# taichi-dev/taichi-nerfs

Hardware: NVIDIA H100
Metric: rays/sec (8192-ray batch, Lego shape) (higher is better)
Workload: dtype f16

## Files before the change

taichi_nerfs_b200/csrc/hash.cu:

```cuda
#include "common.cuh"

namespace {

constexpr int kTile = 512;
constexpr int kChunk = 16;
constexpr int kThreads = 512;
constexpr int kRow = kTile + kTile / kChunk + 1;
constexpr int kXChunk = kChunk + 1;
constexpr int kXWords = (kTile / kChunk) * kXChunk * 4;

struct Dyn {
    const int32_t* n_dev;
    float lo[3], span[3];
    int normalize;
};
__device__ __forceinline__ int64_t effective_n(const Dyn& dyn, int64_t n) {
    if (dyn.n_dev == nullptr) return n;
    const int64_t v = (int64_t)*dyn.n_dev;
    return v < n ? (v < 0 ? 0 : v) : n;
}

struct LevelMeta {
    uint32_t offset;
    uint32_t size;
    uint32_t mask;
    uint32_t res, res2;
    float scale;
    int dense;
};

__device__ __forceinline__ LevelMeta level_meta(const ngp_hash_layout& lay, int l) {
    LevelMeta m;
    m.offset = (uint32_t)lay.offsets[l];
    m.size = (uint32_t)lay.map_sizes[l];
    m.mask = (m.size & (m.size - 1)) == 0 ? m.size - 1 : 0u;
    m.res = lay.resolutions[l];
    m.res2 = m.res * m.res;
    m.scale = lay.scales[l];
    m.dense = l < lay.begin_fast_hash_level;
    return m;
}

template <bool kFracF16>
__device__ __forceinline__ void grid_pos(const float x[3], const LevelMeta& m, uint32_t g[3], float pos[3]) {
#pragma unroll
    for (int d = 0; d < 3; ++d) {
        const float p = f_add(f_mul(x[d], m.scale), 0.5f);
        const float fl = floorf(p);
        g[d] = (uint32_t)(int32_t)fl;
        const float gf = kFracF16 ? __half2float(__float2half_rn((float)g[d])) : (float)g[d];
        pos[d] = f_sub(p, gf);
    }
}

__device__ __forceinline__ void corner_indices(const LevelMeta& m, const uint32_t g[3], uint32_t idx[8]) {
    if (m.dense) {
        const uint32_t base = g[0] + g[1] * m.res + g[2] * m.res2;
#pragma unroll
        for (int c = 0; c < 8; ++c) {
            uint32_t h = base + (c & 1) + ((c >> 1) & 1) * m.res + (c >> 2) * m.res2;
            if (h >= m.size) {
                h -= m.size;
                if (h >= m.size) h %= m.size;
            }
            idx[c] = m.offset + h;
        }
    } else {
        const uint32_t hy0 = g[1] * 2654435761u, hy1 = hy0 + 2654435761u;
        const uint32_t hz0 = g[2] * 805459861u, hz1 = hz0 + 805459861u;
#pragma unroll
        for (int c = 0; c < 8; ++c) {
            const uint32_t h = (g[0] + (c & 1)) ^ ((c & 2) ? hy1 : hy0) ^ ((c & 4) ? hz1 : hz0);
            idx[c] = m.offset + (m.mask ? (h & m.mask) : (h % m.size));
        }
    }
}

__device__ __forceinline__ void corner_weights(const float pos[3], float w[8]) {
    const float ax[2] = {f_sub(1.0f, pos[0]), pos[0]};
    const float ay[2] = {f_sub(1.0f, pos[1]), pos[1]};
    const float az[2] = {f_sub(1.0f, pos[2]), pos[2]};
    float axy[4];
#pragma unroll
    for (int c = 0; c < 4; ++c) axy[c] = f_mul(ax[c & 1], ay[c >> 1]);
#pragma unroll
    for (int c = 0; c < 8; ++c) w[c] = f_mul(axy[c & 3], az[c >> 2]);
}

template <typename T>
struct Vec2;
template <>
struct Vec2<float> { using type = float2; };
template <>
struct Vec2<__half> { using type = __half2; };

template <typename V2>
struct Pair;
template <>
struct Pair<float2> {
    using type = float4;
    __device__ static __forceinline__ float2 lo(const float4& p) { return make_float2(p.x, p.y); }
    __device__ static __forceinline__ float2 hi(const float4& p) { return make_float2(p.z, p.w); }
};
template <>
struct Pair<__half2> {
    using type = uint2;
    __device__ static __forceinline__ __half2 lo(const uint2& p) { return *reinterpret_cast<const __half2*>(&p.x); }
    __device__ static __forceinline__ __half2 hi(const uint2& p) { return *reinterpret_cast<const __half2*>(&p.y); }
};

template <typename T>
__global__ void __launch_bounds__(kThreads) hash_fwd_kernel(const float* __restrict__ xyz,
                                                            const T* __restrict__ table,
                                                            const __grid_constant__ ngp_hash_layout lay,
                                                            T* __restrict__ out, int64_t n_max, const Dyn dyn) {
    using V2 = typename Vec2<T>::type;
    const int64_t n = effective_n(dyn, n_max);
    constexpr bool kHalf = sizeof(T) == 2;
    extern __shared__ __align__(16) uint8_t smem_raw[];
    float* sx = reinterpret_cast<float*>(smem_raw);
    V2* tile = reinterpret_cast<V2*>(smem_raw + kXWords * sizeof(float));

    const int L = lay.n_levels;
    const int64_t base = (int64_t)blockIdx.x * kTile;
    if (base >= n) return;
    const int rows = (int)min((int64_t)kTile, n - base);
    for (int r = threadIdx.x; r < rows; r += kThreads) {
        float v[3];
#pragma unroll
        for (int k = 0; k < 3; ++k) {
            v[k] = xyz[(base + r) * 3 + k];
            if (dyn.normalize) v[k] = f_div(f_sub(v[k], dyn.lo[k]), dyn.span[k]);
        }
        reinterpret_cast<float4*>(sx)[r + r / kChunk] = make_float4(v[0], v[1], v[2], 0.0f);
    }
    __syncthreads();

    const int level = threadIdx.x >> 5, lane = threadIdx.x & 31;
    if (level < L) {
        const LevelMeta m = level_meta(lay, level);
        const V2* tab = reinterpret_cast<const V2*>(table);
        uint32_t pg[3] = {0u, 0u, 0u};
        bool have = false;
        V2 v[8];
        V2* trow = tile + level * kRow + lane * (kChunk + 1);
#pragma unroll 4
        for (int j = 0; j < kChunk; ++j) {
            const int s = lane * kChunk + j;
            if (s >= rows) break;
            const float4 xv = reinterpret_cast<const float4*>(sx)[lane * kXChunk + j];
            const float x[3] = {xv.x, xv.y, xv.z};
            uint32_t g[3];
            float pos[3];
            grid_pos<kHalf>(x, m, g, pos);
            if (!have || g[0] != pg[0] || g[1] != pg[1] || g[2] != pg[2]) {
                have = true;
                uint32_t idx[8];
                corner_indices(m, g, idx);
#pragma unroll
                for (int c = 0; c < 8; c += 2) {
                    if ((idx[c] ^ idx[c + 1]) == 1u) {
                        using V4 = typename Pair<V2>::type;
                        const V4 pr = __ldg(reinterpret_cast<const V4*>(tab + (idx[c] & ~1u)));
                        const V2 lo = Pair<V2>::lo(pr), hi = Pair<V2>::hi(pr);
                        v[c] = (idx[c] & 1u) ? hi : lo;
                        v[c + 1] = (idx[c] & 1u) ? lo : hi;
                    } else {
                        v[c] = __ldg(tab + idx[c]);
                        v[c + 1] = __ldg(tab + idx[c + 1]);
                    }
                }
                pg[0] = g[0];
                pg[1] = g[1];
                pg[2] = g[2];
            }
            float w[8];
            corner_weights(pos, w);
            if constexpr (kHalf) {
                __half2 acc = __float2half2_rn(0.0f);
#pragma unroll
                for (int c = 0; c < 8; ++c) {
                    const float2 t = __half22float2(v[c]);
                    acc = __hadd2(acc, __floats2half2_rn(f_mul(w[c], t.x), f_mul(w[c], t.y)));
                }
                trow[j] = acc;
            } else {
                float2 acc = make_float2(0.0f, 0.0f);
#pragma unroll
                for (int c = 0; c < 8; ++c) {
                    acc.x = f_add(acc.x, f_mul(w[c], v[c].x));
                    acc.y = f_add(acc.y, f_mul(w[c], v[c].y));
                }
                trow[j] = acc;
            }
        }
    }
    __syncthreads();
    V2* o2 = reinterpret_cast<V2*>(out) + base * L;
    constexpr int kVec = 16 / sizeof(V2);
    if (L % kVec == 0 && (reinterpret_cast<uintptr_t>(out) & 15) == 0) {
        const int groups = L / kVec;
        for (int k = threadIdx.x; k < rows * groups; k += kThreads) {
            const int r = k / groups, l0 = (k - r * groups) * kVec;
            V2 v[kVec];
#pragma unroll
            for (int q = 0; q < kVec; ++q) v[q] = tile[(l0 + q) * kRow + r + r / kChunk];
            *reinterpret_cast<uint4*>(o2 + (int64_t)r * L + l0) = *reinterpret_cast<const uint4*>(v);
        }
    } else {
        for (int k = threadIdx.x; k < rows * L; k += kThreads) {
            const int r = k / L, l = k - r * L;
            o2[k] = tile[l * kRow + r + r / kChunk];
        }
    }
}

template <typename T>
__global__ void __launch_bounds__(kThreads) hash_bwd_kernel(const float* __restrict__ xyz,
                                                            const T* __restrict__ dout,
                                                            const __grid_constant__ ngp_hash_layout lay,
                                                            float* __restrict__ grad_table, int64_t n_max,
                                                            const Dyn dyn, int level_begin, int level_end,
                                                            int32_t* __restrict__ found_inf) {
    using V2 = typename Vec2<T>::type;
    const int64_t n = effective_n(dyn, n_max);
    constexpr bool kHalf = sizeof(T) == 2;
    extern __shared__ __align__(16) uint8_t smem_raw[];
    float* sx = reinterpret_cast<float*>(smem_raw);
    V2* tile = reinterpret_cast<V2*>(smem_raw + kXWords * sizeof(float));

    const int L = lay.n_levels;
    const int nthreads = blockDim.x;
    const int64_t base = (int64_t)blockIdx.x * kTile;
    if (base >= n) return;
    const int rows = (int)min((int64_t)kTile, n - base);
    for (int r = threadIdx.x; r < rows; r += nthreads) {
        float v[3];
#pragma unroll
        for (int k = 0; k < 3; ++k) {
            v[k] = xyz[(base + r) * 3 + k];
            if (dyn.normalize) v[k] = f_div(f_sub(v[k], dyn.lo[k]), dyn.span[k]);
        }
        reinterpret_cast<float4*>(sx)[r + r / kChunk] = make_float4(v[0], v[1], v[2], 0.0f);
    }
    const V2* d2 = reinterpret_cast<const V2*>(dout) + base * L;
    constexpr int kVec = 16 / sizeof(V2);
    if (L % kVec == 0 && (reinterpret_cast<uintptr_t>(dout) & 15) == 0) {
        const int groups = L / kVec;
        for (int k = threadIdx.x; k < rows * groups; k += nthreads) {
            const int r = k / groups, l0 = (k - r * groups) * kVec;
            const uint4 raw = __ldg(reinterpret_cast<const uint4*>(d2 + (int64_t)r * L + l0));
            const V2* v = reinterpret_cast<const V2*>(&raw);
#pragma unroll
            for (int q = 0; q < kVec; ++q) tile[(l0 + q) * kRow + r + r / kChunk] = v[q];
        }
    } else {
        for (int k = threadIdx.x; k < rows * L; k += nthreads) {
            const int r = k / L, l = k - r * L;
            tile[l * kRow + r + r / kChunk] = d2[k];
        }
    }
    __syncthreads();

    const int level = level_begin + (threadIdx.x >> 5), lane = threadIdx.x & 31;
    if (level >= L || level >= level_end) return;
    const LevelMeta m = level_meta(lay, level);
    float2* g2 = reinterpret_cast<float2*>(grad_table);
    const V2* trow = tile + level * kRow + lane * (kChunk + 1);

    uint32_t pg[3] = {0u, 0u, 0u};
    float2 acc[8];
    bool pending = false;
    bool bad = false;
    auto flush = [&]() {
        uint32_t idx[8];
        corner_indices(m, pg, idx);
#pragma unroll
        for (int c = 0; c < 8; ++c) bad = bad || !(fabsf(acc[c].x) < INFINITY) || !(fabsf(acc[c].y) < INFINITY);
#pragma unroll
        for (int c = 0; c < 8; c += 2) {
            if ((idx[c] ^ idx[c + 1]) == 1u) {
                const float2 lo = (idx[c] & 1u) ? acc[c + 1] : acc[c], hi = (idx[c] & 1u) ? acc[c] : acc[c + 1];
                atomicAdd(reinterpret_cast<float4*>(g2 + (idx[c] & ~1u)), make_float4(lo.x, lo.y, hi.x, hi.y));
            } else {
                atomicAdd(g2 + idx[c], acc[c]);
                atomicAdd(g2 + idx[c + 1], acc[c + 1]);
            }
        }
    };
#pragma unroll 2
    for (int j = 0; j < kChunk; ++j) {
        const int s = lane * kChunk + j;
        if (s >= rows) break;
        float2 dy;
        if constexpr (kHalf) dy = __half22float2(trow[j]);
        else dy = trow[j];
        if (dy.x == 0.0f && dy.y == 0.0f) continue;
        const float4 xv = reinterpret_cast<const float4*>(sx)[lane * kXChunk + j];
        const float x[3] = {xv.x, xv.y, xv.z};
        uint32_t g[3];
        float pos[3];
        grid_pos<kHalf>(x, m, g, pos);
        if (!pending || g[0] != pg[0] || g[1] != pg[1] || g[2] != pg[2]) {
            if (pending) flush();
            pg[0] = g[0];
            pg[1] = g[1];
            pg[2] = g[2];
#pragma unroll
            for (int c = 0; c < 8; ++c) acc[c] = make_float2(0.0f, 0.0f);
            pending = true;
        }
        float w[8];
        corner_weights(pos, w);
#pragma unroll
        for (int c = 0; c < 8; ++c) {
            acc[c].x += w[c] * dy.x;
            acc[c].y += w[c] * dy.y;
        }
    }
    if (pending) flush();
    if (bad && found_inf != nullptr) *found_inf = 1;
}

template <typename T>
__global__ void __launch_bounds__(256) hash_fwd_generic_kernel(const float* __restrict__ xyz, const T* __restrict__ table,
                                                               const __grid_constant__ ngp_hash_layout lay,
                                                               T* __restrict__ out, int64_t n_max, const Dyn dyn) {
    constexpr bool kHalf = sizeof(T) == 2;
    const int64_t n = effective_n(dyn, n_max);
    const int L = lay.n_levels, F = lay.feat_dim;
    const int64_t gid = (int64_t)blockIdx.x * blockDim.x + threadIdx.x;
    if (gid >= n * L) return;
    const int64_t i = gid / L;
    const int level = (int)(gid - i * L);
    float x[3];
#pragma unroll
    for (int k = 0; k < 3; ++k) {
        x[k] = xyz[i * 3 + k];
        if (dyn.normalize) x[k] = f_div(f_sub(x[k], dyn.lo[k]), dyn.span[k]);
    }
    const LevelMeta m = level_meta(lay, level);
    uint32_t g[3], idx[8];
    float pos[3], w[8];
    grid_pos<kHalf>(x, m, g, pos);
    corner_indices(m, g, idx);
    corner_weights(pos, w);
    for (int f = 0; f < F; ++f) {
        if constexpr (kHalf) {
            __half acc = __float2half_rn(0.0f);
#pragma unroll
            for (int c = 0; c < 8; ++c)
                acc = __hadd(acc, __float2half_rn(f_mul(w[c], __half2float(table[(int64_t)idx[c] * F + f]))));
            out[i * L * F + level * F + f] = acc;
        } else {
            float acc = 0.0f;
#pragma unroll
            for (int c = 0; c < 8; ++c) acc = f_add(acc, f_mul(w[c], table[(int64_t)idx[c] * F + f]));
            out[i * L * F + level * F + f] = acc;
        }
    }
}

template <typename T>
__global__ void __launch_bounds__(256) hash_bwd_generic_kernel(const float* __restrict__ xyz, const T* __restrict__ dout,
                                                               const __grid_constant__ ngp_hash_layout lay,
                                                               float* __restrict__ grad_table, int64_t n_max,
                                                               const Dyn dyn) {
    constexpr bool kHalf = sizeof(T) == 2;
    const int64_t n = effective_n(dyn, n_max);
    const int L = lay.n_levels, F = lay.feat_dim;
    const int64_t gid = (int64_t)blockIdx.x * blockDim.x + threadIdx.x;
    if (gid >= n * L) return;
    const int64_t i = gid / L;
    const int level = (int)(gid - i * L);
    float dy[8];
    bool any = false;
    for (int f = 0; f < F; ++f) {
        dy[f] = load_as_float(dout, i * L * F + level * F + f);
        any |= dy[f] != 0.0f;
    }
    if (!any) return;
    float x[3];
#pragma unroll
    for (int k = 0; k < 3; ++k) {
        x[k] = xyz[i * 3 + k];
        if (dyn.normalize) x[k] = f_div(f_sub(x[k], dyn.lo[k]), dyn.span[k]);
    }
    const LevelMeta m = level_meta(lay, level);
    uint32_t g[3], idx[8];
    float pos[3], w[8];
    grid_pos<kHalf>(x, m, g, pos);
    corner_indices(m, g, idx);
    corner_weights(pos, w);
#pragma unroll
    for (int c = 0; c < 8; ++c)
        for (int f = 0; f < F; ++f) atomicAdd(grad_table + (int64_t)idx[c] * F + f, w[c] * dy[f]);
}

__device__ __forceinline__ uint32_t corner_index(const LevelMeta& m, const uint32_t g[3], int c) {
    uint32_t idx[8];
    corner_indices(m, g, idx);
    return idx[c];
}

template <typename T>
__global__ void __launch_bounds__(256) hash_bwd_input_kernel(const float* __restrict__ xyz,
                                                             const T* __restrict__ table,
                                                             const T* __restrict__ dout,
                                                             const __grid_constant__ ngp_hash_layout lay,
                                                             float* __restrict__ dx, int64_t n) {
    using V2 = typename Vec2<T>::type;
    const int64_t i = (int64_t)blockIdx.x * blockDim.x + threadIdx.x;
    if (i >= n) return;
    const int L = lay.n_levels;
    const float x[3] = {xyz[i * 3 + 0], xyz[i * 3 + 1], xyz[i * 3 + 2]};
    float gx = 0.f, gy = 0.f, gz = 0.f;
    for (int l = 0; l < L; ++l) {
        const LevelMeta m = level_meta(lay, l);
        uint32_t g[3];
        float pos[3];
        grid_pos<false>(x, m, g, pos);
        const V2 dyv = reinterpret_cast<const V2*>(dout)[i * L + l];
        float2 dy;
        if constexpr (sizeof(T) == 2) dy = __half22float2(dyv);
        else dy = dyv;
#pragma unroll
        for (int c = 0; c < 8; ++c) {
            const V2 tv = __ldg(reinterpret_cast<const V2*>(table) + corner_index(m, g, c));
            float2 t;
            if constexpr (sizeof(T) == 2) t = __half22float2(tv);
            else t = tv;
            const float v = (t.x * dy.x + t.y * dy.y) * m.scale;
            const float wx = (c & 1) ? pos[0] : 1.0f - pos[0];
            const float wy = (c & 2) ? pos[1] : 1.0f - pos[1];
            const float wz = (c & 4) ? pos[2] : 1.0f - pos[2];
            gx += ((c & 1) ? v : -v) * wy * wz;
            gy += ((c & 2) ? v : -v) * wx * wz;
            gz += ((c & 4) ? v : -v) * wx * wy;
        }
    }
    dx[i * 3 + 0] = gx;
    dx[i * 3 + 1] = gy;
    dx[i * 3 + 2] = gz;
}

size_t smem_bytes(int n_levels, int vec_bytes) {
    return (size_t)kXWords * sizeof(float) + (size_t)n_levels * kRow * vec_bytes;
}

int configure_smem() {
    static bool done = false;
    if (done) return 0;
    const int big = (int)smem_bytes(NGP_MAX_LEVELS, 8);
    cudaError_t e = cudaFuncSetAttribute(hash_fwd_kernel<float>, cudaFuncAttributeMaxDynamicSharedMemorySize, big);
    if (e == cudaSuccess) e = cudaFuncSetAttribute(hash_bwd_kernel<float>, cudaFuncAttributeMaxDynamicSharedMemorySize, big);
    if (e != cudaSuccess) {
        ngp::set_error("hash kernels: cudaFuncSetAttribute: %s", cudaGetErrorString(e));
        return (int)e;
    }
    done = true;
    return 0;
}

Dyn make_dyn(const int32_t* n_dev, const float* aabb6) {
    Dyn d;
    d.n_dev = n_dev;
    d.normalize = aabb6 != nullptr;
    for (int k = 0; k < 3; ++k) {
        d.lo[k] = aabb6 ? aabb6[k] : 0.0f;
        d.span[k] = aabb6 ? aabb6[3 + k] : 1.0f;
    }
    return d;
}

int check_layout(const ngp_hash_layout* lay) {
    NGP_REQUIRE(lay != nullptr, "null layout");
    NGP_REQUIRE(lay->n_levels >= 1 && lay->n_levels <= NGP_MAX_LEVELS, "n_levels out of range");
    NGP_REQUIRE(lay->feat_dim >= 1 && lay->feat_dim <= 8, "feature_per_level must be in [1, 8]");
    return 0;
}

}

extern "C" {

int ngp_hash_encode_fwd(const float* xyz, const void* table, const ngp_hash_layout* layout, void* out,
                        int dtype, int64_t n, void* stream) {
    return ngp_hash_encode_fwd_dyn(xyz, table, layout, out, dtype, n, nullptr, nullptr, stream);
}

int ngp_hash_encode_fwd_dyn(const float* xyz, const void* table, const ngp_hash_layout* layout, void* out,
                            int dtype, int64_t n, const int32_t* n_dev, const float* aabb6, void* stream) {
    const Dyn dyn = make_dyn(n_dev, aabb6);
    if (int rc = check_layout(layout)) return rc;
    NGP_REQUIRE(n >= 0, "negative n");
    NGP_REQUIRE(dtype == NGP_F32 || dtype == NGP_F16, "bad dtype");
    if (n == 0) return 0;
    NGP_REQUIRE(xyz && table && out, "null pointer");
    cudaStream_t st = ngp::as_stream(stream);
    if (layout->feat_dim != 2) {
        const unsigned gg = (unsigned)((n * layout->n_levels + 255) / 256);
        if (dtype == NGP_F16)
            hash_fwd_generic_kernel<__half><<<gg, 256, 0, st>>>(xyz, (const __half*)table, *layout, (__half*)out, n, dyn);
        else
            hash_fwd_generic_kernel<float><<<gg, 256, 0, st>>>(xyz, (const float*)table, *layout, (float*)out, n, dyn);
        NGP_LAUNCHED("hash_fwd_generic_kernel");
        return 0;
    }
    const unsigned grid = (unsigned)((n + kTile - 1) / kTile);
    if (int rc = configure_smem()) return rc;
    if (dtype == NGP_F16)
        hash_fwd_kernel<__half><<<grid, kThreads, smem_bytes(layout->n_levels, 4), st>>>(xyz, (const __half*)table, *layout, (__half*)out, n, dyn);
    else
        hash_fwd_kernel<float><<<grid, kThreads, smem_bytes(layout->n_levels, 8), st>>>(xyz, (const float*)table, *layout, (float*)out, n, dyn);
    NGP_LAUNCHED("hash_fwd_kernel");
    return 0;
}

int ngp_hash_encode_bwd(const float* xyz, const void* dout, int dout_dtype, const ngp_hash_layout* layout,
                        float* grad_table, int64_t n, void* stream) {
    return ngp_hash_encode_bwd_dyn(xyz, dout, dout_dtype, layout, grad_table, n, nullptr, nullptr, stream);
}

int ngp_hash_encode_bwd_dyn(const float* xyz, const void* dout, int dout_dtype, const ngp_hash_layout* layout,
                            float* grad_table, int64_t n, const int32_t* n_dev, const float* aabb6, void* stream) {
    return ngp_hash_encode_bwd_levels(xyz, dout, dout_dtype, layout, grad_table, n, n_dev, aabb6, 0,
                                      layout ? layout->n_levels : 0, nullptr, stream);
}

int ngp_hash_encode_bwd_levels(const float* xyz, const void* dout, int dout_dtype, const ngp_hash_layout* layout,
                               float* grad_table, int64_t n, const int32_t* n_dev, const float* aabb6, int level_begin,
                               int level_end, int32_t* found_inf_or_null, void* stream) {
    const Dyn dyn = make_dyn(n_dev, aabb6);
    if (int rc = check_layout(layout)) return rc;
    NGP_REQUIRE(level_begin >= 0 && level_begin < level_end && level_end <= layout->n_levels, "bad level range");
    NGP_REQUIRE(n >= 0, "negative n");
    NGP_REQUIRE(dout_dtype == NGP_F32 || dout_dtype == NGP_F16, "bad dtype");
    if (n == 0) return 0;
    NGP_REQUIRE(xyz && dout && grad_table, "null pointer");
    NGP_REQUIRE((reinterpret_cast<uintptr_t>(grad_table) & 7) == 0, "grad_table must be 8-byte aligned");
    cudaStream_t st = ngp::as_stream(stream);
    if (layout->feat_dim != 2) {
        NGP_REQUIRE(level_begin == 0 && level_end == layout->n_levels, "level groups need feature_per_level == 2");
        const unsigned gg = (unsigned)((n * layout->n_levels + 255) / 256);
        if (dout_dtype == NGP_F16)
            hash_bwd_generic_kernel<__half><<<gg, 256, 0, st>>>(xyz, (const __half*)dout, *layout, grad_table, n, dyn);
        else
            hash_bwd_generic_kernel<float><<<gg, 256, 0, st>>>(xyz, (const float*)dout, *layout, grad_table, n, dyn);
        NGP_LAUNCHED("hash_bwd_generic_kernel");
        return 0;
    }
    const unsigned grid = (unsigned)((n + kTile - 1) / kTile);
    if (int rc = configure_smem()) return rc;
    const unsigned threads = 32u * (unsigned)(level_end - level_begin);
    if (dout_dtype == NGP_F16)
        hash_bwd_kernel<__half><<<grid, threads, smem_bytes(layout->n_levels, 4), st>>>(xyz, (const __half*)dout, *layout, grad_table, n, dyn, level_begin, level_end, found_inf_or_null);
    else
        hash_bwd_kernel<float><<<grid, threads, smem_bytes(layout->n_levels, 8), st>>>(xyz, (const float*)dout, *layout, grad_table, n, dyn, level_begin, level_end, found_inf_or_null);
    NGP_LAUNCHED("hash_bwd_kernel");
    return 0;
}

int ngp_hash_encode_bwd_input(const float* xyz, const void* table, const void* dout, int dtype,
                              const ngp_hash_layout* layout, float* dx, int64_t n, void* stream) {
    if (int rc = check_layout(layout)) return rc;
    NGP_REQUIRE(n >= 0, "negative n");
    NGP_REQUIRE(dtype == NGP_F32 || dtype == NGP_F16, "bad dtype");
    if (n == 0) return 0;
    NGP_REQUIRE(xyz && table && dout && dx, "null pointer");
    NGP_REQUIRE(layout->feat_dim == 2, "dL/dx is implemented for feature_per_level == 2");
    const unsigned grid = (unsigned)((n + 255) / 256);
    cudaStream_t st = ngp::as_stream(stream);
    if (dtype == NGP_F16)
        hash_bwd_input_kernel<__half><<<grid, 256, 0, st>>>(xyz, (const __half*)table, (const __half*)dout, *layout, dx, n);
    else
        hash_bwd_input_kernel<float><<<grid, 256, 0, st>>>(xyz, (const float*)table, (const float*)dout, *layout, dx, n);
    NGP_LAUNCHED("hash_bwd_input_kernel");
    return 0;
}

}
```

Before: 2.552 million.

## Split hash backward into L2-sized level groups and carry shared-face gradients

The backward hash-grid kernel now launches a 2D grid. The y dimension covers groups of levels whose gradient tables together fit in about 12 MB, so that atomics from concurrent blocks stay L2-resident; each block handles several row tiles per level to keep the same thread count. When a thread moves to an adjacent cell across a face, the accumulators for the shared corners are carried over instead of being flushed with atomics. Staging loads are batched and use streaming hints. The cost is more complex indexing, extra blocks that exit immediately because the x-grid is still sized by the single tile, and more shared memory per block.

```diff
diff --git a/taichi_nerfs_b200/csrc/hash.cu b/taichi_nerfs_b200/csrc/hash.cu
--- a/taichi_nerfs_b200/csrc/hash.cu
+++ b/taichi_nerfs_b200/csrc/hash.cu
@@ -215,101 +215,148 @@
     }
 }
 
+
+__device__ __forceinline__ void scatter_corners(const LevelMeta& m, const uint32_t g[3], const float2 acc[8],
+                                                float2* __restrict__ g2, bool& bad, uint32_t mask) {
+    uint32_t idx[8];
+    corner_indices(m, g, idx);
+#pragma unroll
+    for (int c = 0; c < 8; ++c)
+        bad = bad || (((mask >> c) & 1u) && (!(fabsf(acc[c].x) < INFINITY) || !(fabsf(acc[c].y) < INFINITY)));
+#pragma unroll
+    for (int c = 0; c < 8; c += 2) {
+        const bool a = (mask >> c) & 1u, b = (mask >> (c + 1)) & 1u;
+        if (a && b && (idx[c] ^ idx[c + 1]) == 1u) {
+            const float2 lo = (idx[c] & 1u) ? acc[c + 1] : acc[c], hi = (idx[c] & 1u) ? acc[c] : acc[c + 1];
+            atomicAdd(reinterpret_cast<float4*>(g2 + (idx[c] & ~1u)), make_float4(lo.x, lo.y, hi.x, hi.y));
+        } else {
+            if (a) atomicAdd(g2 + idx[c], acc[c]);
+            if (b) atomicAdd(g2 + idx[c + 1], acc[c + 1]);
+        }
+    }
+}
+
+__device__ __forceinline__ void leave_cell(const LevelMeta& m, const uint32_t pg[3], const uint32_t g[3], float2 acc[8],
+                                           float2* __restrict__ g2, bool& bad) {
+    const uint32_t dx = g[0] - pg[0], dy = g[1] - pg[1], dz = g[2] - pg[2];
+    const uint32_t d = dx | dy | dz;
+    const bool face = ((dx != 0u) + (dy != 0u) + (dz != 0u)) == 1 && (d == 1u || d == 0xFFFFFFFFu);
+    const int axis = dx ? 0 : (dy ? 1 : 2);
+    const uint32_t with_bit = axis == 0 ? 0xAAu : (axis == 1 ? 0xCCu : 0xF0u);
+    const uint32_t shared = d == 1u ? (0xFFu & ~with_bit) : with_bit;
+    scatter_corners(m, pg, acc, g2, bad, face ? shared : 0xFFu);
+    float2 next[8];
+#pragma unroll
+    for (int c = 0; c < 8; ++c) {
+        const float2 from = axis == 0 ? acc[c ^ 1] : (axis == 1 ? acc[c ^ 2] : acc[c ^ 4]);
+        next[c] = (face && ((shared >> c) & 1u)) ? from : make_float2(0.0f, 0.0f);
+    }
+#pragma unroll
+    for (int c = 0; c < 8; ++c) acc[c] = next[c];
+}
+
+constexpr int kStageBatch = 8;
+
+struct LevelGroups {
+    int first[NGP_MAX_LEVELS + 1];
+};
+
 template <typename T>
 __global__ void __launch_bounds__(kThreads) hash_bwd_kernel(const float* __restrict__ xyz,
                                                             const T* __restrict__ dout,
                                                             const __grid_constant__ ngp_hash_layout lay,
                                                             float* __restrict__ grad_table, int64_t n_max,
-                                                            const Dyn dyn, int level_begin, int level_end,
+                                                            const Dyn dyn,
+                                                            const __grid_constant__ LevelGroups groups,
                                                             int32_t* __restrict__ found_inf) {
     using V2 = typename Vec2<T>::type;
     const int64_t n = effective_n(dyn, n_max);
     constexpr bool kHalf = sizeof(T) == 2;
+    const int L = lay.n_levels;
+    const int level_begin = groups.first[blockIdx.y];
+    const int nthreads = blockDim.x, nl = groups.first[blockIdx.y + 1] - level_begin;
+    const int k = (nthreads >> 5) / nl;
+    const int row_len = k * (kTile + kTile / kChunk) + 1;
     extern __shared__ __align__(16) uint8_t smem_raw[];
     float* sx = reinterpret_cast<float*>(smem_raw);
-    V2* tile = reinterpret_cast<V2*>(smem_raw + kXWords * sizeof(float));
-
-    const int L = lay.n_levels;
-    const int nthreads = blockDim.x;
-    const int64_t base = (int64_t)blockIdx.x * kTile;
+    V2* tile = reinterpret_cast<V2*>(smem_raw + (size_t)k * kXWords * sizeof(float));
+
+    const int64_t base = (int64_t)blockIdx.x * k * kTile;
     if (base >= n) return;
-    const int rows = (int)min((int64_t)kTile, n - base);
-    for (int r = threadIdx.x; r < rows; r += nthreads) {
-        float v[3];
-#pragma unroll
-        for (int k = 0; k < 3; ++k) {
-            v[k] = xyz[(base + r) * 3 + k];
-            if (dyn.normalize) v[k] = f_div(f_sub(v[k], dyn.lo[k]), dyn.span[k]);
-        }
-        reinterpret_cast<float4*>(sx)[r + r / kChunk] = make_float4(v[0], v[1], v[2], 0.0f);
-    }
-    const V2* d2 = reinterpret_cast<const V2*>(dout) + base * L;
-    constexpr int kVec = 16 / sizeof(V2);
-    if (L % kVec == 0 && (reinterpret_cast<uintptr_t>(dout) & 15) == 0) {
-        const int groups = L / kVec;
-        for (int k = threadIdx.x; k < rows * groups; k += nthreads) {
-            const int r = k / groups, l0 = (k - r * groups) * kVec;
-            const uint4 raw = __ldg(reinterpret_cast<const uint4*>(d2 + (int64_t)r * L + l0));
-            const V2* v = reinterpret_cast<const V2*>(&raw);
-#pragma unroll
-            for (int q = 0; q < kVec; ++q) tile[(l0 + q) * kRow + r + r / kChunk] = v[q];
-        }
-    } else {
-        for (int k = threadIdx.x; k < rows * L; k += nthreads) {
-            const int r = k / L, l = k - r * L;
-            tile[l * kRow + r + r / kChunk] = d2[k];
+    const int rows = (int)min((int64_t)k * kTile, n - base);
+    const float* xb = xyz + base * 3;
+    for (int i0 = threadIdx.x; i0 < rows * 3; i0 += nthreads * kStageBatch) {
+        float v[kStageBatch];
+#pragma unroll
+        for (int u = 0; u < kStageBatch; ++u) {
+            const int i = i0 + u * nthreads;
+            if (i < rows * 3) v[u] = __ldcs(xb + i);
+        }
+#pragma unroll
+        for (int u = 0; u < kStageBatch; ++u) {
+            const int i = i0 + u * nthreads;
+            if (i >= rows * 3) break;
+            const int r = i / 3, k = i - 3 * r;
+            float x = v[u];
+            if (dyn.normalize) {
+                const float lo = k == 0 ? dyn.lo[0] : (k == 1 ? dyn.lo[1] : dyn.lo[2]);
+                const float span = k == 0 ? dyn.span[0] : (k == 1 ? dyn.span[1] : dyn.span[2]);
+                x = f_div(f_sub(x, lo), span);
+            }
+            sx[(r + r / kChunk) * 4 + k] = x;
+        }
+    }
+    const V2* d2 = reinterpret_cast<const V2*>(dout) + base * L + level_begin;
+    for (int i0 = threadIdx.x; i0 < rows * nl; i0 += nthreads * kStageBatch) {
+        V2 v[kStageBatch];
+#pragma unroll
+        for (int u = 0; u < kStageBatch; ++u) {
+            const int i = i0 + u * nthreads, r = i / nl;
+            if (i < rows * nl) v[u] = __ldcs(d2 + (int64_t)r * L + (i - r * nl));
+        }
+#pragma unroll
+        for (int u = 0; u < kStageBatch; ++u) {
+            const int i = i0 + u * nthreads, r = i / nl;
+            if (i >= rows * nl) break;
+            tile[(i - r * nl) * row_len + r + r / kChunk] = v[u];
         }
     }
     __syncthreads();
 
-    const int level = level_begin + (threadIdx.x >> 5), lane = threadIdx.x & 31;
-    if (level >= L || level >= level_end) return;
-    const LevelMeta m = level_meta(lay, level);
+    const int warp = threadIdx.x >> 5;
+    if (warp >= nl * k) return;
+    const int chunk = (warp % k) * 32 + (threadIdx.x & 31);
+    const LevelMeta m = level_meta(lay, level_begin + warp / k);
     float2* g2 = reinterpret_cast<float2*>(grad_table);
-    const V2* trow = tile + level * kRow + lane * (kChunk + 1);
+    const V2* trow = tile + (warp / k) * row_len + chunk * (kChunk + 1);
 
     uint32_t pg[3] = {0u, 0u, 0u};
     float2 acc[8];
     bool pending = false;
     bool bad = false;
-    auto flush = [&]() {
-        uint32_t idx[8];
-        corner_indices(m, pg, idx);
-#pragma unroll
-        for (int c = 0; c < 8; ++c) bad = bad || !(fabsf(acc[c].x) < INFINITY) || !(fabsf(acc[c].y) < INFINITY);
-#pragma unroll
-        for (int c = 0; c < 8; c += 2) {
-            if ((idx[c] ^ idx[c + 1]) == 1u) {
-                const float2 lo = (idx[c] & 1u) ? acc[c + 1] : acc[c], hi = (idx[c] & 1u) ? acc[c] : acc[c + 1];
-                atomicAdd(reinterpret_cast<float4*>(g2 + (idx[c] & ~1u)), make_float4(lo.x, lo.y, hi.x, hi.y));
-            } else {
-                atomicAdd(g2 + idx[c], acc[c]);
-                atomicAdd(g2 + idx[c + 1], acc[c + 1]);
-            }
-        }
-    };
 #pragma unroll 2
     for (int j = 0; j < kChunk; ++j) {
-        const int s = lane * kChunk + j;
+        const int s = chunk * kChunk + j;
         if (s >= rows) break;
         float2 dy;
         if constexpr (kHalf) dy = __half22float2(trow[j]);
         else dy = trow[j];
         if (dy.x == 0.0f && dy.y == 0.0f) continue;
-        const float4 xv = reinterpret_cast<const float4*>(sx)[lane * kXChunk + j];
+        const float4 xv = reinterpret_cast<const float4*>(sx)[chunk * kXChunk + j];
         const float x[3] = {xv.x, xv.y, xv.z};
         uint32_t g[3];
         float pos[3];
         grid_pos<kHalf>(x, m, g, pos);
-        if (!pending || g[0] != pg[0] || g[1] != pg[1] || g[2] != pg[2]) {
-            if (pending) flush();
-            pg[0] = g[0];
-            pg[1] = g[1];
-            pg[2] = g[2];
+        if (!pending) {
 #pragma unroll
             for (int c = 0; c < 8; ++c) acc[c] = make_float2(0.0f, 0.0f);
             pending = true;
-        }
+        } else if (g[0] != pg[0] || g[1] != pg[1] || g[2] != pg[2]) {
+            leave_cell(m, pg, g, acc, g2, bad);
+        }
+        pg[0] = g[0];
+        pg[1] = g[1];
+        pg[2] = g[2];
         float w[8];
         corner_weights(pos, w);
 #pragma unroll
@@ -318,7 +365,7 @@
             acc[c].y += w[c] * dy.y;
         }
     }
-    if (pending) flush();
+    if (pending) scatter_corners(m, pg, acc, g2, bad, 0xFFu);
     if (bad && found_inf != nullptr) *found_inf = 1;
 }
 
@@ -448,18 +495,36 @@
     return (size_t)kXWords * sizeof(float) + (size_t)n_levels * kRow * vec_bytes;
 }
 
+size_t bwd_smem_bytes(int nl, int k, int vec_bytes) {
+    return (size_t)k * kXWords * sizeof(float) + (size_t)nl * (k * (kTile + kTile / kChunk) + 1) * vec_bytes;
+}
+
 int configure_smem() {
     static bool done = false;
     if (done) return 0;
     const int big = (int)smem_bytes(NGP_MAX_LEVELS, 8);
     cudaError_t e = cudaFuncSetAttribute(hash_fwd_kernel<float>, cudaFuncAttributeMaxDynamicSharedMemorySize, big);
-    if (e == cudaSuccess) e = cudaFuncSetAttribute(hash_bwd_kernel<float>, cudaFuncAttributeMaxDynamicSharedMemorySize, big);
+    const int big_bwd = (int)bwd_smem_bytes(1, NGP_MAX_LEVELS, 8);
+    if (e == cudaSuccess) e = cudaFuncSetAttribute(hash_bwd_kernel<float>, cudaFuncAttributeMaxDynamicSharedMemorySize, big_bwd);
+    if (e == cudaSuccess) e = cudaFuncSetAttribute(hash_bwd_kernel<__half>, cudaFuncAttributeMaxDynamicSharedMemorySize, big_bwd);
     if (e != cudaSuccess) {
         ngp::set_error("hash kernels: cudaFuncSetAttribute: %s", cudaGetErrorString(e));
         return (int)e;
     }
     done = true;
     return 0;
+}
+
+constexpr int64_t kGroupBytes = 12ll << 20;
+
+int level_group_end(const ngp_hash_layout& lay, int a, int end) {
+    int64_t bytes = (int64_t)lay.map_sizes[a] * lay.feat_dim * 4;
+    int b = a + 1;
+    while (b < end && bytes + (int64_t)lay.map_sizes[b] * lay.feat_dim * 4 <= kGroupBytes) {
+        bytes += (int64_t)lay.map_sizes[b] * lay.feat_dim * 4;
+        ++b;
+    }
+    return b;
 }
 
 Dyn make_dyn(const int32_t* n_dev, const float* aabb6) {
@@ -552,11 +617,28 @@
     }
     const unsigned grid = (unsigned)((n + kTile - 1) / kTile);
     if (int rc = configure_smem()) return rc;
-    const unsigned threads = 32u * (unsigned)(level_end - level_begin);
+    LevelGroups groups{};
+    int n_groups = 0, widest = 1;
+    groups.first[0] = level_begin;
+    for (int a = level_begin; a < level_end; ++n_groups) {
+        const int b = level_group_end(*layout, a, level_end);
+        widest = b - a > widest ? b - a : widest;
+        groups.first[n_groups + 1] = b;
+        a = b;
+    }
+    const int vec = dout_dtype == NGP_F16 ? 4 : 8;
+    size_t smem = 0;
+    for (int g = 0; g < n_groups; ++g) {
+        const int nl = groups.first[g + 1] - groups.first[g];
+        const size_t b = bwd_smem_bytes(nl, widest / nl, vec);
+        smem = b > smem ? b : smem;
+    }
+    const dim3 grid2(grid, (unsigned)n_groups);
+    const unsigned threads = 32u * (unsigned)widest;
     if (dout_dtype == NGP_F16)
-        hash_bwd_kernel<__half><<<grid, threads, smem_bytes(layout->n_levels, 4), st>>>(xyz, (const __half*)dout, *layout, grad_table, n, dyn, level_begin, level_end, found_inf_or_null);
+        hash_bwd_kernel<__half><<<grid2, threads, smem, st>>>(xyz, (const __half*)dout, *layout, grad_table, n, dyn, groups, found_inf_or_null);
     else
-        hash_bwd_kernel<float><<<grid, threads, smem_bytes(layout->n_levels, 8), st>>>(xyz, (const float*)dout, *layout, grad_table, n, dyn, level_begin, level_end, found_inf_or_null);
+        hash_bwd_kernel<float><<<grid2, threads, smem, st>>>(xyz, (const float*)dout, *layout, grad_table, n, dyn, groups, found_inf_or_null);
     NGP_LAUNCHED("hash_bwd_kernel");
     return 0;
 }
```

Result: faster. 2.907 million, median of 6 (+13.9%).
